# excamera/alfalfa

Hardware: AMD Instinct MI355X
Metric: 1080p macroblocks/s decode (bit-exact vs reference) (higher is better)
Workload: dtype u8

## Files before the change

### alfalfa_amd/build.py

```python
import os
import subprocess
import sys

HERE = os.path.dirname(os.path.abspath(__file__))
CSRC = os.path.join(HERE, "csrc")
LIB = os.path.join(HERE, "lib", "libalfalfa_amd.so")
SOURCES = ["parser.cpp", "runtime.cpp", "kernels.hip", "parse_kernels.hip", "quality_kernels.hip", "hash_kernels.hip", "rebase_kernels.hip", "rebase_compact_kernels.hip", "reencode_kernels.hip", "reencode_compact_kernels.hip", "serializer.cpp", "serialize_kernels.hip"]
HEADERS = ["parser.hh", "bool_reader.hh", "parse_common.hh", "tok_fsm.hh", "coeff_pack.hh", "recon_inl.hh", "runtime_types.inc", "runtime_pool.inc", "runtime_tokens.inc", "runtime_records.inc", "runtime_ctx.inc", "runtime_submit.inc", "runtime_decode.inc", "runtime_rasters.inc", "runtime_hashes.inc", "runtime_quality.inc", "runtime_lf_search.inc", "runtime_rebase.inc", "runtime_reencode.inc", "runtime_serialize.inc", "serializer.hh", "serialize_common.hh", "bool_writer.hh", "rebase_inl.hh", "rebase_compact.hh", "reencode_compact.hh", "compact_device.hh", "reencode_search.hh", "reencode_mb.hh", "cost_tables.h", "vp8_tables.h", "vp8_math.hh", "hash_chain.hh", "device_types.h",
           os.path.join("..", "..", "include", "alfalfa_amd.h")]
HIPCC = os.environ.get("HIPCC", "/opt/rocm/bin/hipcc")
FLAGS = ["--offload-arch=gfx950", "-O3", "-std=c++17", "-fPIC", "-shared", "-Wall", "-Wno-unused-function"]


def stale():
    if not os.path.exists(LIB):
        return True
    t = os.path.getmtime(LIB)
    return any(os.path.getmtime(os.path.join(CSRC, f)) > t for f in SOURCES + HEADERS)


def build(force=False, verbose=False):
    if not force and not stale():
        return LIB
    os.makedirs(os.path.dirname(LIB), exist_ok=True)
    cmd = [HIPCC] + FLAGS + os.environ.get("AA_EXTRA_FLAGS", "").split() + [os.path.join(CSRC, s) for s in SOURCES] + ["-o", LIB]
    if verbose:
        print(" ".join(cmd))
    subprocess.run(cmd, check=True)
    return LIB


if __name__ == "__main__":
    build(force="--force" in sys.argv, verbose=True)
    print(LIB)
```

### alfalfa_amd/csrc/parse_kernels.hip

```cpp
#include <hip/hip_runtime.h>

#include <algorithm>

#include "device_types.h"
#include "tok_fsm.hh"
#include "coeff_pack.hh"

#ifndef AA_WORKER_PRIO
#define AA_WORKER_PRIO 3
#endif

namespace {

using aa::ParseJob;

__global__ __launch_bounds__( 64 ) void k_parse_mb_headers( const ParseJob * jobs, const uint32_t * order, int n, int lanes )
{
  __builtin_amdgcn_s_setprio( 2 );

  __shared__ aa::HeaderTables s_tables;
  __shared__ aa::HeaderParams s_params[16];
  const int lane = threadIdx.x;
  for ( uint32_t k = lane; k < sizeof( aa::HeaderTables ) / 4; k += 64 ) reinterpret_cast<uint32_t *>( &s_tables )[k] = reinterpret_cast<const uint32_t *>( &aa::kHeaderTables )[k];
  const int slot = blockIdx.x * lanes + lane;
  const bool mine = lane < lanes && lane < 16 && slot < n;
  const ParseJob * Jp = mine ? &jobs[order[slot]] : nullptr;
  if ( Jp ) {
    const uint32_t * src = reinterpret_cast<const uint32_t *>( static_cast<const aa::HeaderParams *>( &Jp->fp ) );
    for ( uint32_t k = 0; k < sizeof( aa::HeaderParams ) / 4; k++ ) reinterpret_cast<uint32_t *>( &s_params[lane] )[k] = src[k];
  }
  __syncthreads();
  if ( !Jp ) return;
  const ParseJob & J = *Jp;
  if ( J.nmb == 0 ) return;
  const aa::HeaderParams & fp = s_params[lane];
  const aa::HeaderTables & T = s_tables;
  aa::BoolReader32 bd;
  aa::BoolState st; st.bitpos = fp.bd_bitpos; st.range = fp.bd_range; st.active = fp.bd_active;
  bd.resume( J.data + fp.first_off, fp.first_size, st );
  const unsigned mbw = fp.mbw, mbh = fp.mbh;
  const unsigned words_per_row = ( mbw + 63 ) / 64;
  uint32_t intra = 0, split = 0;
  unsigned mi = 0;
  const uint32_t mp_stride = J.mp_stride, mp_base = J.flags_padded, nparts = fp.nparts;
  for ( unsigned row = 0; row < mbh; row++ ) {
    unsigned long long word = 0;
    const uint32_t mp_row = mp_stride ? mp_base + ( row % nparts ) * mp_stride + ( row / nparts ) * mbw : 0u;
    for ( unsigned col = 0; col < mbw; col++, mi++ ) {
      const uint8_t flags = aa::parse_mb_header( bd, fp, T, J.mbs, mi, col, row, static_cast<uint8_t *>( nullptr ) );
      J.mbflags[mi] = flags;
      if ( mp_stride ) J.mbflags[mp_row + col] = flags;
      if ( !( flags & AA_MB_INTER ) ) { intra++; word |= 1ull << ( col & 63 ); }
      else if ( J.mbs[mi].y_mode == aa::SPLITMV ) split = 1;
      if ( ( col & 63 ) == 63 || col + 1 == mbw ) { J.intra_rows[row * words_per_row + ( col >> 6 )] = word; word = 0; }
    }
  }
  J.summary->num_intra_mbs = intra;
  J.summary->has_split = split;
}

__global__ __launch_bounds__( 256 ) void k_segment_fixup( const ParseJob * jobs, const aa_seg_stream * streams, const uint32_t * order )
{
  const aa_seg_stream s = streams[blockIdx.x];
  for ( uint32_t k = 0; k < s.count; k++ ) {
    const uint32_t o = order[s.first + k];
    const ParseJob & J = jobs[o & 0x7FFFFFFFu];
    if ( !J.fp.seg_enabled || J.nmb == 0 ) continue;
    if ( o >> 31 ) {
      for ( uint32_t mi = threadIdx.x; mi < J.nmb; mi += blockDim.x ) s.map[mi] = 3;
      __syncthreads();
    }
    for ( uint32_t mi = threadIdx.x; mi < J.nmb; mi += blockDim.x ) aa::segment_fixup( J.fp, J.mbs[mi], s.map[mi] );
    __syncthreads();
  }
}

struct WorkerArgs {
  aa::TokQueue * q;
  unsigned long long * slots;
  aa::Heap heap;
  uint32_t * exited;
  const uint32_t * retire;
  uint32_t gen;
  uint32_t spread;
  unsigned long long * prof;
  unsigned long long linger_ticks;
  int lanes;
  uint32_t lane_bytes;
  uint32_t mp_hint;
  uint32_t * cu_slots;
  uint32_t cu_cap;
  int16_t * sink;
};

__device__ inline uint32_t queue_take( aa::TokQueue * q, uint32_t want, uint32_t spread, uint32_t * base )
{
  uint32_t h = AA_AT_LOAD( &q->head );
  for ( uint32_t tries = 0; ; tries++ ) {
    const uint32_t avail = AA_AT_LOAD( &q->publish ) - h;
    if ( static_cast<int32_t>( avail ) <= 0 ) return 0;
    const uint32_t share = ( avail + spread - 1u ) / spread;
    const uint32_t n = want < share ? want : share;
    uint32_t expect = h;
    if ( __hip_atomic_compare_exchange_strong( &q->head, &expect, h + n, __ATOMIC_RELAXED, __ATOMIC_RELAXED, __HIP_MEMORY_SCOPE_AGENT ) ) { *base = h; return n; }
    h = expect;
    const uint32_t r = ( blockIdx.x * 2654435761u + tries * 40503u ) >> 27;
    for ( uint32_t k = 0; k <= ( r & ( tries < 4 ? 3u : tries < 8 ? 15u : 31u ) ); k++ ) __builtin_amdgcn_s_sleep( 16 );
    if ( tries > 2048 ) h = AA_AT_LOAD( &q->head );
  }
}

__device__ inline int nth_set_bit( unsigned long long mask, uint32_t n )
{
  for ( uint32_t k = 0; k < n; k++ ) mask &= mask - 1ull;
  return __ffsll( static_cast<long long>( mask ) ) - 1;
}

template <bool PK, bool MP>
__global__ __launch_bounds__( 64 ) void k_token_workers( const WorkerArgs a )
{
  extern __shared__ __attribute__( ( aligned( 16 ) ) ) uint8_t smem[];
  const int lane = threadIdx.x;
#if AA_WORKER_PRIO
  __builtin_amdgcn_s_setprio( AA_WORKER_PRIO );
#endif
  uint32_t cu_slot = 0;
  if ( a.cu_slots ) {
    const uint32_t hw = __builtin_amdgcn_s_getreg( 4 | ( 8 << 6 ) | ( 7 << 11 ) ), xcc = __builtin_amdgcn_s_getreg( 20 | ( 0 << 6 ) | ( 3 << 11 ) );
    cu_slot = ( ( xcc & 15u ) << 8 ) | ( hw & 255u );
    uint32_t before = 0;
    if ( lane == 0 ) before = AA_AT_ADD( &a.cu_slots[cu_slot], 1u );
    before = __shfl( before, 0 );
    if ( before >= a.cu_cap ) {
      if ( lane == 0 ) { AA_AT_ADD( &a.cu_slots[cu_slot], 0xFFFFFFFFu ); AA_AT_ADD( &a.cu_slots[AA_CU_SLOTS - 1], 1u ); AA_AT_ADD( a.exited, 1u ); }
      return;
    }
  }
  for ( uint32_t k = lane; k < aa::tok::kTablesBytes / 4; k += 64 ) reinterpret_cast<uint32_t *>( smem )[k] = aa::tok::table_word( k );
  __syncthreads();
  aa::tok::Lane L;
  aa::tok::Frame F {};
  const bool is_lane = lane < a.lanes;
  aa::tok::init_lane( L, aa::tok::ring_addr( is_lane ? lane : 0 ), aa::tok::slice_addr( is_lane ? lane : 0, a.lanes, a.lane_bytes ),
                      (AA_GLOBAL int16_t *) ( a.sink + ( blockIdx.x & 63u ) * 32u + ( lane & 31 ) ) );
  aa::tok::preload( L, smem );
  uint32_t backoff = 0;
  unsigned long long idle_since = 0;
  uint32_t looks = 0;
  bool retiring = false;
  aa::tok::PeriodProf pp { 0, 0, 0 };
  unsigned long long p_look = 0, p_topup = 0, p_period = 0, p_lanes = 0, p_periods = 0;
  const bool profiling = a.prof != nullptr;
  const auto prof_flush = [&]() {
    __hip_atomic_fetch_add( &a.prof[0], pp.pass_ticks, __ATOMIC_RELAXED, __HIP_MEMORY_SCOPE_AGENT );
    __hip_atomic_fetch_add( &a.prof[1], pp.passes, __ATOMIC_RELAXED, __HIP_MEMORY_SCOPE_AGENT );
    __hip_atomic_fetch_add( &a.prof[2], pp.steps, __ATOMIC_RELAXED, __HIP_MEMORY_SCOPE_AGENT );
    __hip_atomic_fetch_add( &a.prof[3], p_look, __ATOMIC_RELAXED, __HIP_MEMORY_SCOPE_AGENT );
    __hip_atomic_fetch_add( &a.prof[4], p_topup, __ATOMIC_RELAXED, __HIP_MEMORY_SCOPE_AGENT );
    __hip_atomic_fetch_add( &a.prof[5], p_period, __ATOMIC_RELAXED, __HIP_MEMORY_SCOPE_AGENT );
    __hip_atomic_fetch_add( &a.prof[6], p_lanes, __ATOMIC_RELAXED, __HIP_MEMORY_SCOPE_AGENT );
    __hip_atomic_fetch_add( &a.prof[7], p_periods, __ATOMIC_RELAXED, __HIP_MEMORY_SCOPE_AGENT );
  };
  for ( ;; ) {
    const unsigned long long t_a = profiling ? wall_clock64() : 0ull;
    const bool idle = is_lane && L.rec == aa::tok::R_DONE;
    const unsigned long long idle_mask = __ballot( idle );
    bool looked = false;
    if ( idle_mask && !retiring ) {
      if ( backoff ) backoff--;
      else {
        looked = true;
        const int first = __ffsll( static_cast<long long>( idle_mask ) ) - 1;
        uint32_t base = 0, got = 0;
        if ( lane == first ) {
          if ( ( looks++ & 7u ) == 0 && __hip_atomic_load( a.retire, __ATOMIC_RELAXED, __HIP_MEMORY_SCOPE_SYSTEM ) >= a.gen ) got = 0xFFFFFFFFu;
          else {
            uint32_t want = static_cast<uint32_t>( __popcll( idle_mask ) );
            if constexpr ( MP ) want = want / a.mp_hint > 1u ? want / a.mp_hint : 1u;
            got = queue_take( a.q, want, a.spread, &base );
          }
        }
        base = __shfl( base, first ); got = __shfl( got, first );
        if ( got == 0xFFFFFFFFu ) { retiring = true; got = 0; }
        const uint32_t rank = static_cast<uint32_t>( __popcll( idle_mask & ( ( 1ull << lane ) - 1ull ) ) );
        const bool mine = idle && rank < got;
        if ( got ) {
          __builtin_amdgcn_fence( __ATOMIC_ACQUIRE, "agent" );
          const aa::ParseJob * job = nullptr;
          if ( mine ) job = reinterpret_cast<const aa::ParseJob *>( AA_AT_LOAD( &a.slots[( base + rank ) & a.q->mask] ) );
          if constexpr ( MP ) {
            const uint32_t n_idle = static_cast<uint32_t>( __popcll( idle_mask ) );
            const int my_parts = mine ? static_cast<int>( job->nmb && job->mp_stride ? job->fp.nparts : 1u ) : 1;
            const aa::tok::MpDeal d = aa::tok::mp_deal( n_idle, got, rank, [&]( uint32_t t ) {
              return static_cast<uint32_t>( __shfl( my_parts, nth_set_bit( idle_mask, t ) ) ); } );
            const long long jp = __shfl( static_cast<long long>( reinterpret_cast<uintptr_t>( job ) ), nth_set_bit( idle_mask, d.ticket ) );
            if ( idle && d.any ) {
              const aa::ParseJob * my_job = reinterpret_cast<const aa::ParseJob *>( static_cast<uintptr_t>( jp ) );
              if ( d.n > 1u ) {
                const int owner_lane = nth_set_bit( idle_mask, d.start + aa::tok::mp_owner_partition( my_job ) );
                F = aa::tok::frame_of_partition( my_job, d.part, aa::tok::slice_addr( owner_lane, a.lanes, a.lane_bytes ) );
              } else F = aa::tok::frame_of( my_job );
              if ( my_job->nmb == 0 ) { L.rec = aa::tok::R_DONE; aa::tok::preload( L, smem ); }
              else aa::tok::begin_frame<MP>( L, smem, L.base, F );
            }
          } else if ( mine ) {
            F = aa::tok::frame_of( job );
            if ( F.nmb == 0 ) { L.rec = aa::tok::R_DONE; aa::tok::preload( L, smem ); }
            else aa::tok::begin_frame<MP>( L, smem, L.base, F );
          }
        } else backoff = 3;
      }
    }
    const bool active = is_lane && L.rec != aa::tok::R_DONE;
    if ( !__any( active ) ) {
      if ( retiring ) break;
      if ( looked ) {
        const unsigned long long now = wall_clock64();
        if ( !idle_since ) idle_since = now | 1ull;
        else if ( now - idle_since > a.linger_ticks ) break;
        for ( int k = 0; k < 16; k++ ) __builtin_amdgcn_s_sleep( 127 );
      }
      backoff = 0;
      continue;
    }
    idle_since = 0;
    const unsigned long long t_b = profiling ? wall_clock64() : 0ull;
    if ( active ) aa::tok::top_up<MP>( L, smem, F );
    const unsigned long long t_c = profiling ? wall_clock64() : 0ull;
    aa::tok::run_period<PK, MP>( L, smem, F, a.heap, profiling, pp );
    if ( profiling ) {
      const unsigned long long t_d = wall_clock64();
      p_look += t_b - t_a; p_topup += t_c - t_b; p_period += t_d - t_c;
      p_lanes += static_cast<unsigned long long>( __popcll( __ballot( active ) ) ); p_periods++;
      if ( ( p_periods & 1023ull ) == 0 ) {
        if ( lane == 0 ) prof_flush();
        pp = { 0, 0, 0 }; p_look = p_topup = p_period = p_lanes = p_periods = 0;
      }
    }
  }
  if ( lane == 0 ) {
    if ( profiling ) prof_flush();
    if ( a.cu_slots ) AA_AT_ADD( &a.cu_slots[cu_slot], 0xFFFFFFFFu );
    AA_AT_ADD( a.exited, 1u );
  }
}

__global__ __launch_bounds__( 64 ) void k_enqueue_jobs( aa::TokQueue * q, unsigned long long * slots, const ParseJob * jobs, const uint32_t * order, int n )
{
  __shared__ uint32_t s_base;
  if ( threadIdx.x == 0 ) s_base = AA_AT_ADD( &q->reserve, static_cast<uint32_t>( n ) );
  __syncthreads();
  const uint32_t base = s_base, mask = q->mask;
  for ( int i = threadIdx.x; i < n; i += 64 ) AA_AT_STORE( &slots[( base + i ) & mask], reinterpret_cast<unsigned long long>( &jobs[order[i]] ) );
  __syncthreads();
  if ( threadIdx.x == 0 ) {
    __builtin_amdgcn_fence( __ATOMIC_RELEASE, "agent" );
    asm volatile( "s_waitcnt vmcnt(0)" ::: "memory" );
    while ( AA_AT_LOAD( &q->publish ) != base ) __builtin_amdgcn_s_sleep( 8 );
    AA_AT_STORE( &q->publish, base + static_cast<uint32_t>( n ) );
  }
}

__device__ inline void pool_push_wave( const aa::Heap & H, const AA_GLOBAL uint32_t * ids, uint32_t first, uint32_t n_mine )
{
  __shared__ uint32_t s_off[65];
  __shared__ uint32_t s_pbase;
  s_off[threadIdx.x + 1] = n_mine;
  __syncthreads();
  if ( threadIdx.x == 0 ) {
    s_off[0] = 0;
    for ( int i = 1; i <= 64; i++ ) s_off[i] += s_off[i - 1];
    s_pbase = s_off[64] ? AA_AT_ADD( &H.pool->reserve, s_off[64] ) : 0u;
  }
  __syncthreads();
  const uint32_t b = s_pbase + s_off[threadIdx.x], mask = H.pool->mask, total = s_off[64];
  for ( uint32_t i = 0; i < n_mine; i++ ) AA_AT_STORE( &H.ring[( b + i ) & mask], ids ? ids[i] : first + i );
  __syncthreads();
  if ( threadIdx.x == 0 && total ) {
    __builtin_amdgcn_fence( __ATOMIC_RELEASE, "agent" );
    asm volatile( "s_waitcnt vmcnt(0)" ::: "memory" );
    while ( AA_AT_LOAD( &H.pool->publish ) != s_pbase ) __builtin_amdgcn_s_sleep( 8 );
    AA_AT_STORE( &H.pool->publish, s_pbase + total );
    AA_AT_ADD_REL( &H.pool->avail, static_cast<int32_t>( total ) );
  }
}
__global__ __launch_bounds__( 64 ) void k_pool_push_range( aa::Heap heap, uint32_t first, uint32_t count )
{
  const uint32_t per = ( count + 63u ) / 64u, lo = threadIdx.x * per;
  const uint32_t mine = lo >= count ? 0u : ( count - lo < per ? count - lo : per );
  pool_push_wave( heap, nullptr, first + lo, mine );
}
struct FreeLists { const uint32_t * l[AA_MAX_BATCH]; };
__global__ __launch_bounds__( 64 ) void k_pool_free_lists( aa::Heap heap, const FreeLists lists, int n )
{
  const int i = blockIdx.x * 64 + threadIdx.x;
  const AA_GLOBAL uint32_t * l = ( i < n && lists.l[i] ) ? (const AA_GLOBAL uint32_t *) lists.l[i] : nullptr;
  pool_push_wave( heap, l ? l + 1 : nullptr, 0, l ? l[0] : 0u );
}
__global__ void k_mirror_counters( const aa::TokQueue * q, const aa::CoeffPool * pool, const uint32_t * exited, int n_grids, const unsigned long long * prof, aa_tok_mirror * out, uint32_t seq )
{
  if ( threadIdx.x || blockIdx.x ) return;
  if ( prof ) for ( int k = 0; k < 8; k++ ) out->prof[k] = AA_AT_LOAD( &prof[k] );
  out->q_head = AA_AT_LOAD( &q->head ); out->q_publish = AA_AT_LOAD( &q->publish ); out->q_reserve = AA_AT_LOAD( &q->reserve );
  if ( pool ) { out->pool_avail = AA_AT_LOAD( &pool->avail ); out->pool_starving = AA_AT_LOAD( &pool->starving ); }
  for ( int g = 0; g < n_grids; g++ ) out->exited[g] = AA_AT_LOAD( &exited[g] );
  __builtin_amdgcn_fence( __ATOMIC_RELEASE, "" );
  asm volatile( "s_waitcnt vmcnt(0)" ::: "memory" );
  __hip_atomic_store( &out->seq, seq, __ATOMIC_RELAXED, __HIP_MEMORY_SCOPE_SYSTEM );
}

}

namespace aa {

static int parse_lanes_env()
{
  static const int lanes = [] {
    const char * e = getenv( "ALFALFA_AMD_PARSE_LANES" );
    const int v = e ? atoi( e ) : 0;
    return v < 0 ? 0 : ( v > 64 ? 64 : v );
  }();
  return lanes;
}
static int header_lanes() { const int v = parse_lanes_env(); return v ? std::min( v, 16 ) : 16; }

constexpr uint32_t kLdsPerCu = 160u * 1024u, kLdsGranule = 512u;
static uint32_t env_u32( const char * name, uint32_t dflt ) { const char * e = getenv( name ); return e ? static_cast<uint32_t>( atoi( e ) ) : dflt; }
static const uint32_t kWgsPerCu = std::max( 1u, std::min( 16u, env_u32( "ALFALFA_AMD_WGS_PER_CU", 3u ) ) );
static const uint32_t kMaxLanes = std::max( 1u, std::min( 64u, env_u32( "ALFALFA_AMD_MAX_LANES", 30u ) ) );
struct TokenShape { int lanes; uint32_t lds; int per_cu; };
static TokenShape token_launch_shape( uint32_t lane_bytes )
{
  for ( uint32_t n = kWgsPerCu; n >= 1; n-- ) {
    const uint32_t request = std::min( 65536u, ( kLdsPerCu / ( n + 1 ) / kLdsGranule + 1 ) * kLdsGranule );
    if ( request < tok::kTablesBytes + lane_bytes || request * n > kLdsPerCu ) continue;
    const int lanes = static_cast<int>( std::min<uint32_t>( kMaxLanes, ( request - tok::kTablesBytes ) / lane_bytes ) );
    return { lanes, request, static_cast<int>( n ) };
  }
  return { 0, 0, 0 };
}

int launch_parse_mb_headers( const ParseJob * jobs, const uint32_t * order, int n, void * stream )
{
  const int lanes = header_lanes();
  hipLaunchKernelGGL( k_parse_mb_headers, dim3( ( n + lanes - 1 ) / lanes ), dim3( 64 ), 0, static_cast<hipStream_t>( stream ), jobs, order, n, lanes );
  return static_cast<int>( hipGetLastError() );
}

int launch_segment_fixup( const ParseJob * jobs, const aa_seg_stream * streams, int n_streams, const uint32_t * order, void * stream )
{
  hipLaunchKernelGGL( k_segment_fixup, dim3( n_streams ), dim3( 256 ), 0, static_cast<hipStream_t>( stream ), jobs, streams, order );
  return static_cast<int>( hipGetLastError() );
}

void token_worker_shape( uint32_t lane_bytes, int n_cus, int * lanes_out, uint32_t * lds_out, int * wgs_per_cu_out )
{
  int lanes = parse_lanes_env();
  uint32_t lds = 0;
  if ( lanes ) {
    if ( static_cast<uint32_t>( lanes ) * lane_bytes + tok::kTablesBytes > 65536u ) lanes = static_cast<int>( ( 65536u - tok::kTablesBytes ) / lane_bytes );
    lds = static_cast<uint32_t>( lanes ) * lane_bytes + tok::kTablesBytes;
  } else {
    const TokenShape sh = token_launch_shape( lane_bytes );
    lanes = sh.lanes; lds = sh.lds;
  }
  (void) n_cus;
  static const bool lds_exact = env_u32( "ALFALFA_AMD_LDS_EXACT", 1u ) != 0u;
  static const uint32_t wgs_cap = env_u32( "ALFALFA_AMD_WGS_CAP_PER_CU", lds_exact && !parse_lanes_env() ? kWgsPerCu : 0u );
  if ( lds_exact && lanes > 0 ) lds = ( ( tok::kTablesBytes + static_cast<uint32_t>( lanes ) * lane_bytes + kLdsGranule - 1u ) / kLdsGranule ) * kLdsGranule;
  *lanes_out = lanes; *lds_out = lds;
  int per_cu = lds ? static_cast<int>( kLdsPerCu / lds ) : 0;
  if ( wgs_cap && per_cu > static_cast<int>( wgs_cap ) ) per_cu = static_cast<int>( wgs_cap );
  *wgs_per_cu_out = per_cu;
}

int launch_token_workers( TokQueue * q, unsigned long long * slots, const Heap & heap, uint32_t * exited, const uint32_t * retire, uint32_t gen, uint32_t spread,
                          unsigned long long * prof, unsigned long long linger_ticks, int wgs, int lanes, uint32_t lane_bytes, uint32_t lds, bool packed, uint32_t mp_hint, void * stream,
                          uint32_t * cu_slots, uint32_t cu_cap )
{
  if ( lanes < 1 || wgs < 1 ) return static_cast<int>( hipErrorInvalidValue );
  WorkerArgs a;
  a.q = q; a.slots = slots; a.heap = heap; a.exited = exited; a.retire = retire; a.gen = gen; a.spread = spread ? spread : 1u; a.prof = prof; a.linger_ticks = linger_ticks; a.lanes = lanes; a.lane_bytes = lane_bytes;
  a.mp_hint = mp_hint ? mp_hint : 1u;
  a.cu_slots = cu_cap ? cu_slots : nullptr; a.cu_cap = cu_cap;
  a.sink = reinterpret_cast<int16_t *>( cu_slots + AA_CU_SLOTS / 2 );
  if ( mp_hint ) {
    if ( packed ) hipLaunchKernelGGL( ( k_token_workers<true, true> ), dim3( wgs ), dim3( 64 ), lds, static_cast<hipStream_t>( stream ), a );
    else hipLaunchKernelGGL( ( k_token_workers<false, true> ), dim3( wgs ), dim3( 64 ), lds, static_cast<hipStream_t>( stream ), a );
  } else {
    if ( packed ) hipLaunchKernelGGL( ( k_token_workers<true, false> ), dim3( wgs ), dim3( 64 ), lds, static_cast<hipStream_t>( stream ), a );
    else hipLaunchKernelGGL( ( k_token_workers<false, false> ), dim3( wgs ), dim3( 64 ), lds, static_cast<hipStream_t>( stream ), a );
  }
  return static_cast<int>( hipGetLastError() );
}

int launch_enqueue_jobs( TokQueue * q, unsigned long long * slots, const ParseJob * jobs, const uint32_t * order, int n, void * stream )
{
  hipLaunchKernelGGL( k_enqueue_jobs, dim3( 1 ), dim3( 64 ), 0, static_cast<hipStream_t>( stream ), q, slots, jobs, order, n );
  return static_cast<int>( hipGetLastError() );
}

int launch_pool_push_range( const Heap & heap, uint32_t first, uint32_t count, void * stream )
{
  hipLaunchKernelGGL( k_pool_push_range, dim3( 1 ), dim3( 64 ), 0, static_cast<hipStream_t>( stream ), heap, first, count );
  return static_cast<int>( hipGetLastError() );
}

int launch_pool_free_lists( const Heap & heap, const uint32_t * const * lists, int n, void * stream )
{
  for ( int base = 0; base < n; base += AA_MAX_BATCH ) {
    FreeLists fl;
    const int cnt = std::min( AA_MAX_BATCH, n - base );
    for ( int i = 0; i < AA_MAX_BATCH; i++ ) fl.l[i] = i < cnt ? lists[base + i] : nullptr;
    hipLaunchKernelGGL( k_pool_free_lists, dim3( ( cnt + 63 ) / 64 ), dim3( 64 ), 0, static_cast<hipStream_t>( stream ), heap, fl, cnt );
    if ( hipError_t e = hipGetLastError() ) return static_cast<int>( e );
  }
  return 0;
}

int launch_mirror_counters( const TokQueue * q, const CoeffPool * pool, const uint32_t * exited, int n_grids, const unsigned long long * prof, aa_tok_mirror * out, uint32_t seq, void * stream )
{
  hipLaunchKernelGGL( k_mirror_counters, dim3( 1 ), dim3( 64 ), 0, static_cast<hipStream_t>( stream ), q, pool, exited, n_grids, prof, out, seq );
  return static_cast<int>( hipGetLastError() );
}

}
```

Measured before the change: 125.0 million.

## Rewrite MB header parse kernel with register-resident neighbour state and packed tables

Replaces the generic per-lane header parser with a device-specialised version. It keeps above/left neighbour info in registers, prefetching the next above record. It packs probability tables into words, reads the bitstream through a 16-byte chunked bool reader, and writes whole 16-byte MB records plus gathered 4-byte flag stores. The goal is fewer scattered global loads and stores and fewer LDS parameter copies in this serial, latency-bound kernel. The cost is a large amount of duplicated parsing logic that must stay bit-exact with the reference parser.

```diff
diff --git a/alfalfa_amd/build.py b/alfalfa_amd/build.py
--- a/alfalfa_amd/build.py
+++ b/alfalfa_amd/build.py
@@ -6,7 +6,7 @@
 CSRC = os.path.join(HERE, "csrc")
 LIB = os.path.join(HERE, "lib", "libalfalfa_amd.so")
 SOURCES = ["parser.cpp", "runtime.cpp", "kernels.hip", "parse_kernels.hip", "quality_kernels.hip", "hash_kernels.hip", "rebase_kernels.hip", "rebase_compact_kernels.hip", "reencode_kernels.hip", "reencode_compact_kernels.hip", "serializer.cpp", "serialize_kernels.hip"]
-HEADERS = ["parser.hh", "bool_reader.hh", "parse_common.hh", "tok_fsm.hh", "coeff_pack.hh", "recon_inl.hh", "runtime_types.inc", "runtime_pool.inc", "runtime_tokens.inc", "runtime_records.inc", "runtime_ctx.inc", "runtime_submit.inc", "runtime_decode.inc", "runtime_rasters.inc", "runtime_hashes.inc", "runtime_quality.inc", "runtime_lf_search.inc", "runtime_rebase.inc", "runtime_reencode.inc", "runtime_serialize.inc", "serializer.hh", "serialize_common.hh", "bool_writer.hh", "rebase_inl.hh", "rebase_compact.hh", "reencode_compact.hh", "compact_device.hh", "reencode_search.hh", "reencode_mb.hh", "cost_tables.h", "vp8_tables.h", "vp8_math.hh", "hash_chain.hh", "device_types.h",
+HEADERS = ["parser.hh", "bool_reader.hh", "parse_common.hh", "parse_device.hh", "tok_fsm.hh", "coeff_pack.hh", "recon_inl.hh", "runtime_types.inc", "runtime_pool.inc", "runtime_tokens.inc", "runtime_records.inc", "runtime_ctx.inc", "runtime_submit.inc", "runtime_decode.inc", "runtime_rasters.inc", "runtime_hashes.inc", "runtime_quality.inc", "runtime_lf_search.inc", "runtime_rebase.inc", "runtime_reencode.inc", "runtime_serialize.inc", "serializer.hh", "serialize_common.hh", "bool_writer.hh", "rebase_inl.hh", "rebase_compact.hh", "reencode_compact.hh", "compact_device.hh", "reencode_search.hh", "reencode_mb.hh", "cost_tables.h", "vp8_tables.h", "vp8_math.hh", "hash_chain.hh", "device_types.h",
            os.path.join("..", "..", "include", "alfalfa_amd.h")]
 HIPCC = os.environ.get("HIPCC", "/opt/rocm/bin/hipcc")
 FLAGS = ["--offload-arch=gfx950", "-O3", "-std=c++17", "-fPIC", "-shared", "-Wall", "-Wno-unused-function"]
diff --git a/alfalfa_amd/csrc/parse_device.hh b/alfalfa_amd/csrc/parse_device.hh
--- /dev/null
+++ b/alfalfa_amd/csrc/parse_device.hh
@@ -0,0 +1,450 @@
+#pragma once
+#include "tok_fsm.hh"
+
+namespace aa {
+namespace hdr {
+
+struct alignas( 16 ) DevTables {
+  uint32_t kf_b_mode_probs[100][3];
+  uint32_t b_mode_probs[3];
+  uint8_t mv_counts_to_probs[24];
+  uint8_t submv_ref_probs[5][4];
+  uint8_t kf_y_mode_probs[4], kf_uv_mode_probs[4], split_mv_probs[4];
+};
+static_assert( sizeof( DevTables ) % 16 == 0, "DevTables is copied as words" );
+constexpr DevTables make_dev_tables()
+{
+  DevTables t {};
+  for ( int c = 0; c < 100; c++ ) for ( int k = 0; k < 9; k++ ) t.kf_b_mode_probs[c][k >> 2] |= static_cast<uint32_t>( k_kf_b_mode_probs[c * 9 + k] ) << ( 8 * ( k & 3 ) );
+  for ( int k = 0; k < 9; k++ ) t.b_mode_probs[k >> 2] |= static_cast<uint32_t>( k_b_mode_probs[k] ) << ( 8 * ( k & 3 ) );
+  for ( int k = 0; k < 24; k++ ) t.mv_counts_to_probs[k] = k_mv_counts_to_probs[k];
+  for ( int c = 0; c < 5; c++ ) for ( int k = 0; k < 3; k++ ) t.submv_ref_probs[c][k] = k_submv_ref_probs[c * 3 + k];
+  for ( int k = 0; k < 4; k++ ) t.kf_y_mode_probs[k] = k_kf_y_mode_probs[k];
+  for ( int k = 0; k < 3; k++ ) { t.kf_uv_mode_probs[k] = k_kf_uv_mode_probs[k]; t.split_mv_probs[k] = k_split_mv_probs[k]; }
+  return t;
+}
+constexpr DevTables kDevTables = make_dev_tables();
+
+constexpr uint32_t kMvStride = 20;
+struct alignas( 4 ) LaneTables { uint8_t mv_probs[2][kMvStride]; };
+
+constexpr uint64_t pack_b_tree( int from, int to )
+{
+  uint64_t r = 0;
+  for ( int e = from; e < to; e++ ) {
+    const int v = kBModeTree[e];
+    r |= static_cast<uint64_t>( v > 0 ? v : ( 32 - v ) ) << ( 6 * ( e - from ) );
+  }
+  return r;
+}
+constexpr uint64_t kBTreeLo = pack_b_tree( 0, 10 ), kBTreeHi = pack_b_tree( 10, 18 );
+
+AA_HD inline uint32_t byte_of( uint32_t w, uint32_t k ) { return ( w >> ( 8u * k ) ) & 0xFFu; }
+
+struct DirectMem {
+  static AA_HD inline V16 stream16( uintptr_t a ) { return *reinterpret_cast<const AA_GLOBAL V16 *>( a ); }
+  static AA_HD inline uint32_t load4( uintptr_t a ) { return *reinterpret_cast<const AA_GLOBAL uint32_t *>( a ); }
+  static AA_HD inline V8 load8( uintptr_t a ) { return *reinterpret_cast<const AA_GLOBAL V8 *>( a ); }
+  static AA_HD inline void store16( uintptr_t a, const V16 & v ) { *reinterpret_cast<AA_GLOBAL V16 *>( a ) = v; }
+  static AA_HD inline void store8( uintptr_t a, unsigned long long v ) { *reinterpret_cast<AA_GLOBAL unsigned long long *>( a ) = v; }
+  static AA_HD inline void store4( uintptr_t a, uint32_t v ) { *reinterpret_cast<AA_GLOBAL uint32_t *>( a ) = v; }
+  static AA_HD inline void store1( uintptr_t a, uint32_t v ) { *reinterpret_cast<AA_GLOBAL uint8_t *>( a ) = static_cast<uint8_t>( v ); }
+};
+
+template <class Mem>
+class BoolReader16
+{
+  uintptr_t chunk0_ = 0, idle_ = 0;
+  uint32_t next_ = 0, lim_ = 0;
+  int left_ = 0;
+  uint32_t q0_ = 0, q1_ = 0, q2_ = 0, q3_ = 0, nq_ = 0;
+  uint32_t w_ = 0, nb_ = 0;
+  uint32_t value_ = 0;
+  int count_ = 0;
+  uint32_t range_ = 255;
+
+  AA_HD inline uint32_t next_word()
+  {
+    if ( nq_ == 0 ) {
+      const V16 c = Mem::stream16( next_ < lim_ ? chunk0_ + next_ : idle_ );
+      q0_ = c.x; q1_ = c.y; q2_ = c.z; q3_ = c.w; nq_ = 4;
+      next_ += 16;
+    }
+    const uint32_t w = q0_;
+    q0_ = q1_; q1_ = q2_; q2_ = q3_; nq_--;
+    return w;
+  }
+  AA_HD inline uint32_t next_byte()
+  {
+    if ( nb_ == 0 ) { w_ = next_word(); nb_ = 4; }
+    const uint32_t byte = left_ > 0 ? ( w_ & 0xFFu ) : 0u;
+    w_ >>= 8; nb_--; left_--;
+    return byte;
+  }
+
+public:
+  AA_HD BoolReader16() {}
+  AA_HD void resume( const uint8_t * base, uint32_t size, const BoolState & st, uintptr_t idle )
+  {
+    const uintptr_t b = reinterpret_cast<uintptr_t>( base ), a = b + ( st.bitpos >> 3 );
+    const uint32_t r = st.bitpos & 7;
+    idle_ = idle;
+    chunk0_ = a & ~static_cast<uintptr_t>( 15 );
+    const long long lim = static_cast<long long>( b + size ) - static_cast<long long>( chunk0_ );
+    lim_ = lim > 0 ? static_cast<uint32_t>( lim ) : 0u;
+    left_ = static_cast<int>( size ) - static_cast<int>( st.bitpos >> 3 );
+    range_ = st.range;
+    next_ = 0; nq_ = 0;
+    for ( uint32_t k = static_cast<uint32_t>( a >> 2 ) & 3u; k; k-- ) next_word();
+    w_ = next_word() >> ( 8u * static_cast<uint32_t>( a & 3u ) ); nb_ = 4u - static_cast<uint32_t>( a & 3u );
+    uint32_t bits = 0;
+    for ( int k = 0; k < 3; k++ ) bits = ( bits << 8 ) | next_byte();
+    value_ = ( static_cast<uint32_t>( st.active ) << 24 ) | ( ( bits << r ) & 0xFFFFFFu );
+    count_ = 24 - static_cast<int>( r );
+  }
+  AA_HD inline int get( const uint32_t prob )
+  {
+    const uint32_t split = 1 + ( ( ( range_ - 1 ) * prob ) >> 8 );
+    if ( count_ < 0 ) {
+      value_ |= next_byte() << ( 16 - count_ );
+      count_ += 8;
+    }
+    const uint32_t bigsplit = split << 24;
+    int bit;
+    uint32_t range;
+    if ( value_ >= bigsplit ) { range = range_ - split; value_ -= bigsplit; bit = 1; }
+    else { range = split; bit = 0; }
+    const int shift = __builtin_clz( range ) - 24;
+    range_ = range << shift;
+    value_ <<= shift;
+    count_ -= shift;
+    return bit;
+  }
+};
+
+struct Neighbour { uint32_t w0 = 0, w1 = 0, t = 0; };
+
+AA_HD inline uint32_t pack_mv( Mv m ) { return static_cast<uint16_t>( m.x ) | ( static_cast<uint32_t>( static_cast<uint16_t>( m.y ) ) << 16 ); }
+AA_HD inline Mv unpack_mv( uint32_t p ) { Mv m; m.x = static_cast<int16_t>( p & 0xFFFFu ); m.y = static_cast<int16_t>( p >> 16 ); return m; }
+AA_HD inline uint32_t negate_mv( uint32_t p ) { return ( ( 0u - p ) & 0xFFFFu ) | ( ( 0u - ( p >> 16 ) ) << 16 ); }
+AA_HD inline uint32_t add_mv( uint32_t a, uint32_t b ) { return ( ( a + b ) & 0xFFFFu ) | ( ( ( a >> 16 ) + ( b >> 16 ) ) << 16 ); }
+
+struct Census { uint32_t s0 = 0, s1 = 0, s2 = 0, s3 = 0, c1 = 0, c2 = 0, c3 = 0, idx = 0, split = 0; };
+
+struct LaneParams {
+  uint32_t mbw, mbh;
+  uint32_t probs;
+  uint32_t y_mode_probs, uv_mode_probs, seg_tree_probs;
+  uint32_t fadj_ref, fadj_mode;
+  uint32_t seg_level_lo, seg_level_hi;
+  bool key, seg_update, skip_enabled, flip_golden, flip_alt, lf_on, fadj_on;
+};
+template <class P>
+AA_HD inline LaneParams lane_params( P fp )
+{
+  LaneParams L;
+  L.mbw = fp->mbw; L.mbh = fp->mbh;
+  L.probs = fp->prob_skip | ( fp->prob_inter << 8 ) | ( fp->prob_last << 16 ) | ( static_cast<uint32_t>( fp->prob_golden ) << 24 );
+  L.y_mode_probs = fp->y_mode_probs[0] | ( fp->y_mode_probs[1] << 8 ) | ( fp->y_mode_probs[2] << 16 ) | ( static_cast<uint32_t>( fp->y_mode_probs[3] ) << 24 );
+  L.uv_mode_probs = fp->uv_mode_probs[0] | ( fp->uv_mode_probs[1] << 8 ) | ( fp->uv_mode_probs[2] << 16 );
+  L.seg_tree_probs = fp->seg_tree_probs[0] | ( fp->seg_tree_probs[1] << 8 ) | ( fp->seg_tree_probs[2] << 16 );
+  L.fadj_ref = L.fadj_mode = 0;
+  for ( int k = 0; k < 4; k++ ) {
+    L.fadj_ref |= static_cast<uint32_t>( static_cast<uint8_t>( fp->fadj_ref[k] ) ) << ( 8 * k );
+    L.fadj_mode |= static_cast<uint32_t>( static_cast<uint8_t>( fp->fadj_mode[k] ) ) << ( 8 * k );
+  }
+  L.seg_level_lo = static_cast<uint16_t>( fp->seg_level[0] ) | ( static_cast<uint32_t>( static_cast<uint16_t>( fp->seg_level[1] ) ) << 16 );
+  L.seg_level_hi = static_cast<uint16_t>( fp->seg_level[2] ) | ( static_cast<uint32_t>( static_cast<uint16_t>( fp->seg_level[3] ) ) << 16 );
+  L.key = fp->key != 0; L.seg_update = fp->seg_enabled && fp->seg_update_map; L.skip_enabled = fp->skip_enabled != 0;
+  L.flip_golden = fp->sign_bias_golden != 0; L.flip_alt = fp->sign_bias_alt != 0;
+  L.lf_on = fp->loop_filter_level != 0; L.fadj_on = fp->fadj_enabled != 0;
+  return L;
+}
+
+AA_HD inline bool lane_mv_flipped( const LaneParams & L, uint32_t ref_frame )
+{
+  return ( ref_frame == GOLDEN_FRAME && L.flip_golden ) || ( ref_frame == ALTREF_FRAME && L.flip_alt );
+}
+
+AA_HD inline Census consider( Census C, const LaneParams & L, bool my_flip, const Neighbour & nb, bool there, uint32_t weight )
+{
+  const bool counts = there && ( nb.w1 & AA_MB_INTER );
+  uint32_t mv = nb.t;
+  if ( lane_mv_flipped( L, byte_of( nb.w0, 2 ) ) != my_flip ) mv = negate_mv( mv );
+  const bool zero = mv == 0;
+  const uint32_t cur = C.idx == 1 ? C.c1 : ( C.idx == 2 ? C.c2 : ( C.idx == 3 ? C.c3 : 0u ) );
+  const uint32_t idx = C.idx + ( counts && !zero && mv != cur ? 1u : 0u );
+  const bool cand = counts && !zero;
+  Census R = C;
+  R.idx = idx;
+  R.s0 += counts && zero ? weight : 0u;
+  R.s1 += cand && idx == 1 ? weight : 0u; R.c1 = cand && idx == 1 ? mv : C.c1;
+  R.s2 += cand && idx == 2 ? weight : 0u; R.c2 = cand && idx == 2 ? mv : C.c2;
+  R.s3 += cand && idx == 3 ? weight : 0u; R.c3 = cand && idx == 3 ? mv : C.c3;
+  R.split += counts && byte_of( nb.w0, 0 ) == SPLITMV ? weight : 0u;
+  return R;
+}
+
+AA_HD inline uint32_t lane_lf_level( const LaneParams & L, uint32_t segment_id, uint32_t ref_frame, uint32_t y_mode )
+{
+  if ( !L.lf_on ) return 0;
+  const uint32_t pair = segment_id & 2u ? L.seg_level_hi : L.seg_level_lo;
+  int level = static_cast<int16_t>( segment_id & 1u ? pair >> 16 : pair & 0xFFFFu );
+  if ( L.fadj_on ) {
+    level += static_cast<int8_t>( byte_of( L.fadj_ref, ref_frame ) );
+    uint32_t k = 2;
+    if ( ref_frame == CURRENT_FRAME ) k = 0;
+    else if ( y_mode == ZEROMV ) k = 1;
+    else if ( y_mode == SPLITMV ) k = 3;
+    if ( ref_frame != CURRENT_FRAME || y_mode == B_PRED ) level += static_cast<int8_t>( byte_of( L.fadj_mode, k ) );
+  }
+  return static_cast<uint32_t>( level <= 0 ? 0 : ( level > 63 ? 63 : level ) );
+}
+
+template <class BD>
+AA_HD inline uint32_t read_b_mode( BD & bd, uint32_t pa, uint32_t pb, uint32_t pc )
+{
+  uint32_t i = 0;
+  for ( ;; ) {
+    const uint32_t node = i >> 1;
+    const uint32_t word = node < 4 ? pa : ( node < 8 ? pb : pc );
+    const uint32_t e = i + static_cast<uint32_t>( bd.get( byte_of( word, node & 3u ) ) );
+    const uint32_t code = static_cast<uint32_t>( e < 10 ? kBTreeLo >> ( 6u * e ) : kBTreeHi >> ( 6u * ( e - 10u ) ) ) & 63u;
+    if ( code & 32u ) return code & 31u;
+    i = code;
+  }
+}
+
+template <class BD>
+AA_HD inline uint32_t read_mv_component_dev( BD & bd, const uint8_t * p )
+{
+  enum { MV_IS_SHORT, SIGN, SHORT, BITS = SHORT + 8 - 1, MV_LONG_BITS = 10 };
+  int x = 0;
+  if ( bd.get( p[MV_IS_SHORT] ) ) {
+    unsigned long long order = 0x456789210ull;
+#if defined( __HIP_DEVICE_COMPILE__ )
+#pragma nounroll
+#endif
+    for ( int k = 0; k < 9; k++, order >>= 4 ) { const int i = static_cast<int>( order & 15u ); x += bd.get( p[BITS + i] ) << i; }
+    if ( !( x & 0xFFF0 ) || bd.get( p[BITS + 3] ) ) x += 8;
+  } else {
+    const int b0 = bd.get( p[SHORT] );
+    const int b1 = bd.get( p[SHORT + 1 + 3 * b0] );
+    const int b2 = bd.get( p[SHORT + 2 + 3 * b0 + b1] );
+    x = ( b0 << 2 ) | ( b1 << 1 ) | b2;
+  }
+  x <<= 1;
+  if ( x && bd.get( p[SIGN] ) ) x = -x;
+  return static_cast<uint32_t>( x ) & 0xFFFFu;
+}
+template <class BD>
+AA_HD inline uint32_t read_mv_dev( BD & bd, const LaneTables & LT )
+{
+  uint32_t m = 0;
+#if defined( __HIP_DEVICE_COMPILE__ )
+#pragma nounroll
+#endif
+  for ( uint32_t c = 0; c < 2; c++ ) m = ( m << 16 ) | read_mv_component_dev( bd, LT.mv_probs[c] );
+  return m;
+}
+
+template <class Mem>
+struct FlagGather {
+  uint32_t acc = 0, n = 0;
+  AA_HD inline void put( uintptr_t base, uint32_t idx, uint32_t flags, bool last_of_run )
+  {
+    const uint32_t pos = idx & 3u;
+    acc |= flags << ( 8u * pos ); n++;
+    if ( pos == 3u || last_of_run ) {
+      if ( n == 4u ) Mem::store4( base + idx - 3u, acc );
+      else for ( uint32_t k = 0; k < n; k++ ) Mem::store1( base + idx - ( n - 1u ) + k, byte_of( acc, pos - ( n - 1u ) + k ) );
+      acc = 0; n = 0;
+    }
+  }
+};
+
+template <class P>
+AA_HD inline void fill_lane_tables( LaneTables & LT, P fp )
+{
+  for ( uint32_t c = 0; c < 2; c++ ) for ( uint32_t k = 0; k < kMvStride; k++ ) LT.mv_probs[c][k] = k < 19 ? fp->mv_probs[c][k] : 0;
+}
+
+template <class Mem, class JobPtr>
+AA_HD inline void parse_frame_headers( JobPtr J, const DevTables & T, const LaneTables & LT )
+{
+  const LaneParams L = lane_params( &J->fp );
+  const uint32_t mbw = L.mbw, mbh = L.mbh, nmb = mbw * mbh;
+  const uintptr_t mbs = reinterpret_cast<uintptr_t>( J->mbs ), mbflags = reinterpret_cast<uintptr_t>( J->mbflags );
+  const uintptr_t intra_rows = reinterpret_cast<uintptr_t>( J->intra_rows );
+  const uint32_t mp_stride = J->mp_stride, mp_base = J->flags_padded, nparts = J->fp.nparts;
+  BoolReader16<Mem> bd;
+  {
+    BoolState st; st.bitpos = J->fp.bd_bitpos; st.range = J->fp.bd_range; st.active = J->fp.bd_active;
+    bd.resume( reinterpret_cast<const uint8_t *>( reinterpret_cast<uintptr_t>( J->data ) + J->fp.first_off ), J->fp.first_size, st, reinterpret_cast<uintptr_t>( J ) );
+  }
+  const uint32_t words_per_row = ( mbw + 63u ) / 64u;
+  const uint32_t nb_tail = L.key ? 28u : 76u;
+  const bool key = L.key;
+  uint32_t intra = 0, split = 0, mi = 0;
+  Neighbour above, above_left, left;
+  FlagGather<Mem> raster, by_partition;
+  for ( uint32_t row = 0; row < mbh; row++ ) {
+    unsigned long long word = 0;
+    const uint32_t mp_row = mp_stride ? mp_base + ( row % nparts ) * mp_stride + ( row / nparts ) * mbw : 0u;
+    for ( uint32_t col = 0; col < mbw; col++, mi++ ) {
+      const uintptr_t nb_at = mbs + static_cast<uintptr_t>( mi + 1u >= mbw ? mi + 1u - mbw : 0u ) * sizeof( aa_mb_info );
+      const V8 next_head = Mem::load8( nb_at );
+      const uint32_t next_tail = Mem::load4( nb_at + nb_tail );
+
+      uint32_t segment_id = 0;
+      if ( L.seg_update ) {
+        if ( !bd.get( byte_of( L.seg_tree_probs, 0 ) ) ) segment_id = static_cast<uint32_t>( bd.get( byte_of( L.seg_tree_probs, 1 ) ) );
+        else segment_id = 2u + static_cast<uint32_t>( bd.get( byte_of( L.seg_tree_probs, 2 ) ) );
+      }
+      const bool skip = L.skip_enabled ? bd.get( byte_of( L.probs, 0 ) ) != 0 : false;
+      bool inter = false;
+      uint32_t ref_frame = CURRENT_FRAME;
+      if ( !key ) {
+        inter = bd.get( byte_of( L.probs, 1 ) ) != 0;
+        if ( inter ) {
+          ref_frame = LAST_FRAME;
+          if ( bd.get( byte_of( L.probs, 2 ) ) ) ref_frame = bd.get( byte_of( L.probs, 3 ) ) ? ALTREF_FRAME : GOLDEN_FRAME;
+        }
+      }
+
+      uint32_t y_mode, uv_mode = 0, split_partition = 0, flags = 0;
+      uint32_t u0, u1, u2, u3, u4, u5, u6, u7, u8, u9, u10, u11, u12, u13, u14, u15;
+      if ( !inter ) {
+        if ( key ) {
+          if ( !bd.get( T.kf_y_mode_probs[0] ) ) y_mode = B_PRED;
+          else if ( !bd.get( T.kf_y_mode_probs[1] ) ) y_mode = bd.get( T.kf_y_mode_probs[2] ) ? V_PRED : DC_PRED;
+          else y_mode = bd.get( T.kf_y_mode_probs[3] ) ? TM_PRED : H_PRED;
+        } else {
+          if ( !bd.get( byte_of( L.y_mode_probs, 0 ) ) ) y_mode = DC_PRED;
+          else if ( !bd.get( byte_of( L.y_mode_probs, 1 ) ) ) y_mode = bd.get( byte_of( L.y_mode_probs, 2 ) ) ? H_PRED : V_PRED;
+          else y_mode = bd.get( byte_of( L.y_mode_probs, 3 ) ) ? B_PRED : TM_PRED;
+        }
+        if ( y_mode == B_PRED ) {
+          const uint32_t left_col = key && col > 0 ? left.t : 0u;
+          uint32_t prev_row = key && row > 0 ? above.t : 0u, cur = 0;
+          const uint32_t * fixed = T.b_mode_probs;
+          u0 = u1 = u2 = u3 = 0;
+#if defined( __HIP_DEVICE_COMPILE__ )
+#pragma nounroll
+#endif
+          for ( uint32_t b = 0; b < 16; b++ ) {
+            const uint32_t c = b & 3u;
+            const uint32_t * p = fixed;
+            if ( key ) {
+              const uint32_t above_mode = byte_of( prev_row, c ), left_mode = c ? byte_of( cur, c - 1u ) : byte_of( left_col, b >> 2 );
+              p = T.kf_b_mode_probs[above_mode * 10u + left_mode];
+            }
+            cur |= read_b_mode( bd, p[0], p[1], p[2] ) << ( 8u * c );
+            if ( c == 3u ) { u0 = u1; u1 = u2; u2 = u3; u3 = cur; prev_row = cur; cur = 0; }
+          }
+        } else {
+          const uint32_t implied = ( ( static_cast<uint32_t>( B_TM_PRED ) << 24 ) | ( B_HE_PRED << 16 ) | ( B_VE_PRED << 8 ) | B_DC_PRED ) >> ( 8u * y_mode ) & 0xFFu;
+          u0 = u1 = u2 = u3 = implied * 0x01010101u;
+        }
+        u4 = u5 = u6 = u7 = u8 = u9 = u10 = u11 = u12 = u13 = u14 = u15 = 0;
+        const uint32_t uvp = key ? ( T.kf_uv_mode_probs[0] | ( T.kf_uv_mode_probs[1] << 8 ) | ( T.kf_uv_mode_probs[2] << 16 ) ) : L.uv_mode_probs;
+        if ( !bd.get( byte_of( uvp, 0 ) ) ) uv_mode = DC_PRED;
+        else if ( !bd.get( byte_of( uvp, 1 ) ) ) uv_mode = V_PRED;
+        else uv_mode = bd.get( byte_of( uvp, 2 ) ) ? TM_PRED : H_PRED;
+      } else {
+        flags |= AA_MB_INTER;
+        const bool my_flip = lane_mv_flipped( L, ref_frame );
+        Census C;
+        C = consider( C, L, my_flip, above, row > 0, 2 );
+        C = consider( C, L, my_flip, left, col > 0, 2 );
+        C = consider( C, L, my_flip, above_left, row > 0 && col > 0, 1 );
+        uint32_t s0 = C.s0, s1 = C.s1, s2 = C.s2, c0 = 0, c1 = C.c1, c2 = C.c2;
+        const uint32_t s3 = C.s3, c3 = C.c3, split_score = C.split;
+        if ( s3 && c3 == c1 ) s1 += s3;
+        if ( s2 > s1 ) { const uint32_t ts = s1; s1 = s2; s2 = ts; const uint32_t tc = c1; c1 = c2; c2 = tc; }
+        if ( s1 >= s0 ) c0 = c1;
+        const uint32_t p0 = T.mv_counts_to_probs[s0 * 4 + 0], p1 = T.mv_counts_to_probs[s1 * 4 + 1],
+                       p2 = T.mv_counts_to_probs[s2 * 4 + 2], p3 = T.mv_counts_to_probs[split_score * 4 + 3];
+        if ( !bd.get( p0 ) ) y_mode = ZEROMV;
+        else if ( !bd.get( p1 ) ) y_mode = NEARESTMV;
+        else if ( !bd.get( p2 ) ) y_mode = NEARMV;
+        else y_mode = bd.get( p3 ) ? SPLITMV : NEWMV;
+        if ( y_mode != SPLITMV ) {
+          uint32_t base = 0;
+          if ( y_mode == NEARESTMV ) base = pack_mv( clamp_mv( unpack_mv( c1 ), col, row, mbw, mbh ) );
+          else if ( y_mode == NEARMV ) base = pack_mv( clamp_mv( unpack_mv( c2 ), col, row, mbw, mbh ) );
+          else if ( y_mode == NEWMV ) base = add_mv( read_mv_dev( bd, LT ), pack_mv( clamp_mv( unpack_mv( c0 ), col, row, mbw, mbh ) ) );
+          u0 = u1 = u2 = u3 = u4 = u5 = u6 = u7 = u8 = u9 = u10 = u11 = u12 = u13 = u14 = u15 = base;
+        } else {
+          if ( !bd.get( T.split_mv_probs[0] ) ) split_partition = 3;
+          else if ( !bd.get( T.split_mv_probs[1] ) ) split_partition = 2;
+          else split_partition = bd.get( T.split_mv_probs[2] ) ? 1 : 0;
+          const uint32_t first_mask = ( 0xFA28u >> ( 4u * split_partition ) ) & 15u;
+          const uint32_t best = pack_mv( clamp_mv( unpack_mv( c0 ), col, row, mbw, mbh ) );
+          const bool left_inter = col > 0 && ( left.w1 & AA_MB_INTER ), above_inter = row > 0 && ( above.w1 & AA_MB_INTER );
+          const bool left_split = left_inter && byte_of( left.w0, 0 ) == SPLITMV, above_split = above_inter && byte_of( above.w0, 0 ) == SPLITMV;
+          const uintptr_t left_mv = mbs + static_cast<uintptr_t>( mi - ( col > 0 ? 1u : 0u ) ) * sizeof( aa_mb_info ) + 16u;
+          const uintptr_t above_mv = mbs + static_cast<uintptr_t>( mi - ( row > 0 ? mbw : 0u ) ) * sizeof( aa_mb_info ) + 16u;
+          uint32_t h0 = 0, h1 = 0, h2 = 0, h3 = 0, h4 = 0, h5 = 0, h6 = 0, h7 = 0, h8 = 0, h9 = 0, h10 = 0, h11 = 0, h12 = 0, h13 = 0, h14 = 0, h15 = 0;
+#if defined( __HIP_DEVICE_COMPILE__ )
+#pragma nounroll
+#endif
+          for ( uint32_t b = 0; b < 16; b++ ) {
+            const uint32_t rest = b & ~first_mask & 15u;
+            uint32_t m;
+            if ( rest == 0 ) {
+              uint32_t lmv, amv;
+              if ( b & 3u ) lmv = h0;
+              else lmv = left_split ? Mem::load4( left_mv + 4u * ( b + 3u ) ) : ( left_inter ? left.t : 0u );
+              if ( b >= 4u ) amv = h3;
+              else amv = above_split ? Mem::load4( above_mv + 4u * ( b + 12u ) ) : ( above_inter ? above.t : 0u );
+              uint32_t ctx = 0;
+              if ( lmv == amv ) ctx = lmv == 0 ? 4 : 3;
+              else if ( amv == 0 ) ctx = 2;
+              else if ( lmv == 0 ) ctx = 1;
+              const uint8_t * sp = T.submv_ref_probs[ctx];
+              if ( !bd.get( sp[0] ) ) m = lmv;
+              else if ( !bd.get( sp[1] ) ) m = amv;
+              else if ( !bd.get( sp[2] ) ) m = 0;
+              else m = add_mv( read_mv_dev( bd, LT ), best );
+            } else m = ( rest & 3u ) ? h0 : h3;
+            h15 = h14; h14 = h13; h13 = h12; h12 = h11; h11 = h10; h10 = h9; h9 = h8; h8 = h7;
+            h7 = h6; h6 = h5; h5 = h4; h4 = h3; h3 = h2; h2 = h1; h1 = h0; h0 = m;
+          }
+          u0 = h15; u1 = h14; u2 = h13; u3 = h12; u4 = h11; u5 = h10; u6 = h9; u7 = h8;
+          u8 = h7; u9 = h6; u10 = h5; u11 = h4; u12 = h3; u13 = h2; u14 = h1; u15 = h0;
+          split = 1;
+        }
+      }
+
+      if ( !( y_mode == B_PRED || y_mode == SPLITMV ) ) flags |= AA_MB_HAS_Y2;
+      if ( skip ) flags |= AA_MB_SKIP;
+      const uint32_t lf_level = lane_lf_level( L, segment_id, ref_frame, y_mode );
+      const uint32_t w0 = y_mode | ( uv_mode << 8 ) | ( ref_frame << 16 ) | ( segment_id << 24 );
+      const uint32_t w1 = flags | ( lf_level << 8 ) | ( split_partition << 16 );
+
+      Neighbour me; me.w0 = w0; me.w1 = w1;
+      me.t = key ? ( ( u0 >> 24 ) | ( ( u1 >> 24 ) << 8 ) | ( ( u2 >> 24 ) << 16 ) | ( u3 & 0xFF000000u ) ) : u15;
+      above_left = above;
+      if ( mbw > 1u ) { above.w0 = next_head.x; above.w1 = next_head.y; above.t = next_tail; }
+      else { above = me; if ( key ) above.t = u3; }
+      left = me;
+
+      const uintptr_t rec = mbs + static_cast<uintptr_t>( mi ) * sizeof( aa_mb_info );
+      Mem::store16( rec, V16 { w0, w1, 0u, 0u } );
+      Mem::store16( rec + 16, V16 { u0, u1, u2, u3 } );
+      Mem::store16( rec + 32, V16 { u4, u5, u6, u7 } );
+      Mem::store16( rec + 48, V16 { u8, u9, u10, u11 } );
+      Mem::store16( rec + 64, V16 { u12, u13, u14, u15 } );
+      raster.put( mbflags, mi, flags, mi + 1u == nmb );
+      if ( mp_stride ) by_partition.put( mbflags, mp_row + col, flags, col + 1u == mbw );
+      if ( !( flags & AA_MB_INTER ) ) { intra++; word |= 1ull << ( col & 63u ); }
+      if ( ( col & 63u ) == 63u || col + 1u == mbw ) { Mem::store8( intra_rows + 8u * ( row * words_per_row + ( col >> 6 ) ), word ); word = 0; }
+    }
+  }
+  Mem::store4( reinterpret_cast<uintptr_t>( &J->summary->num_intra_mbs ), intra );
+  Mem::store4( reinterpret_cast<uintptr_t>( &J->summary->has_split ), split );
+}
+
+}
+}
diff --git a/alfalfa_amd/csrc/parse_kernels.hip b/alfalfa_amd/csrc/parse_kernels.hip
--- a/alfalfa_amd/csrc/parse_kernels.hip
+++ b/alfalfa_amd/csrc/parse_kernels.hip
@@ -4,6 +4,7 @@
 
 #include "device_types.h"
 #include "tok_fsm.hh"
+#include "parse_device.hh"
 #include "coeff_pack.hh"
 
 #ifndef AA_WORKER_PRIO
@@ -18,45 +19,17 @@
 {
   __builtin_amdgcn_s_setprio( 2 );
 
-  __shared__ aa::HeaderTables s_tables;
-  __shared__ aa::HeaderParams s_params[16];
+  __shared__ aa::hdr::DevTables s_tables;
+  __shared__ aa::hdr::LaneTables s_lane[16];
   const int lane = threadIdx.x;
-  for ( uint32_t k = lane; k < sizeof( aa::HeaderTables ) / 4; k += 64 ) reinterpret_cast<uint32_t *>( &s_tables )[k] = reinterpret_cast<const uint32_t *>( &aa::kHeaderTables )[k];
+  for ( uint32_t k = lane; k < sizeof( aa::hdr::DevTables ) / 4; k += 64 ) reinterpret_cast<uint32_t *>( &s_tables )[k] = reinterpret_cast<const uint32_t *>( &aa::hdr::kDevTables )[k];
   const int slot = blockIdx.x * lanes + lane;
   const bool mine = lane < lanes && lane < 16 && slot < n;
-  const ParseJob * Jp = mine ? &jobs[order[slot]] : nullptr;
-  if ( Jp ) {
-    const uint32_t * src = reinterpret_cast<const uint32_t *>( static_cast<const aa::HeaderParams *>( &Jp->fp ) );
-    for ( uint32_t k = 0; k < sizeof( aa::HeaderParams ) / 4; k++ ) reinterpret_cast<uint32_t *>( &s_params[lane] )[k] = src[k];
-  }
-  __syncthreads();
-  if ( !Jp ) return;
-  const ParseJob & J = *Jp;
-  if ( J.nmb == 0 ) return;
-  const aa::HeaderParams & fp = s_params[lane];
-  const aa::HeaderTables & T = s_tables;
-  aa::BoolReader32 bd;
-  aa::BoolState st; st.bitpos = fp.bd_bitpos; st.range = fp.bd_range; st.active = fp.bd_active;
-  bd.resume( J.data + fp.first_off, fp.first_size, st );
-  const unsigned mbw = fp.mbw, mbh = fp.mbh;
-  const unsigned words_per_row = ( mbw + 63 ) / 64;
-  uint32_t intra = 0, split = 0;
-  unsigned mi = 0;
-  const uint32_t mp_stride = J.mp_stride, mp_base = J.flags_padded, nparts = fp.nparts;
-  for ( unsigned row = 0; row < mbh; row++ ) {
-    unsigned long long word = 0;
-    const uint32_t mp_row = mp_stride ? mp_base + ( row % nparts ) * mp_stride + ( row / nparts ) * mbw : 0u;
-    for ( unsigned col = 0; col < mbw; col++, mi++ ) {
-      const uint8_t flags = aa::parse_mb_header( bd, fp, T, J.mbs, mi, col, row, static_cast<uint8_t *>( nullptr ) );
-      J.mbflags[mi] = flags;
-      if ( mp_stride ) J.mbflags[mp_row + col] = flags;
-      if ( !( flags & AA_MB_INTER ) ) { intra++; word |= 1ull << ( col & 63 ); }
-      else if ( J.mbs[mi].y_mode == aa::SPLITMV ) split = 1;
-      if ( ( col & 63 ) == 63 || col + 1 == mbw ) { J.intra_rows[row * words_per_row + ( col >> 6 )] = word; word = 0; }
-    }
-  }
-  J.summary->num_intra_mbs = intra;
-  J.summary->has_split = split;
+  const AA_GLOBAL ParseJob * J = mine ? (const AA_GLOBAL ParseJob *) &jobs[order[slot]] : nullptr;
+  if ( J ) aa::hdr::fill_lane_tables( s_lane[lane], &J->fp );
+  __syncthreads();
+  if ( !J || J->nmb == 0 ) return;
+  aa::hdr::parse_frame_headers<aa::hdr::DirectMem>( J, s_tables, s_lane[lane] );
 }
 
 __global__ __launch_bounds__( 256 ) void k_segment_fixup( const ParseJob * jobs, const aa_seg_stream * streams, const uint32_t * order )
```

Result: slower. 122.6 million (-1.9%).
